# ulab-uiuc/UniRec

Hardware: AMD Instinct MI355X
Metric: user-sequences/sec joint fwd+bwd (Qwen3-0.6B+LoRA, hist=50) (higher is better)
Workload: dtype bf16; 1 GPU; C4 joint step: item Q-Former(L12,H1024,Q2,F14) on 64x50 items -> inject -> Qwen3-0.6B-shaped(28L)+LoRA r16 -> mean-pool -> InfoNCE pool 1000; fwd+bwd+allreduce+AdamW; per_gpu_batch=64, global_batch=64, seq_len=2048, hist=50, pool=1000, micro_batches=1, recompute_mlp=False, parallelism=dp1, random_init=True

## Files before the change

unirec_amd/csrc/gemm.hip:

```cpp
#include <cstdlib>
#include <type_traits>
#include "common.hip.h"
#include "unirec_hip.h"
#include "gemm_common.hip.h"

using urgemm::GemmP;
using urgemm::GemmPlan;
using urgemm::GemmGroups;
using urgemm::GemmGroupSlot;
using urgemm::UR_GEMM_MAX_GROUPS;
using urgemm::uniform_ptr;

namespace {

#ifndef UR_GEMM_STAMPS
#define UR_GEMM_STAMPS 0
#endif
#if UR_GEMM_STAMPS
__device__ long long g_gemm_stamps[8192 * 8];
#define UR_STAMP(k) do { if (threadIdx.x == 0 && blockIdx.x < 8192 && blockIdx.z == 0) g_gemm_stamps[blockIdx.x * 8 + (k)] = (long long)__builtin_readcyclecounter(); } while (0)
#else
#define UR_STAMP(k) do { } while (0)
#endif
constexpr int BK = 64;
// ... 218 lines not shown
    float4 a = w4[i];
    for (int z = 1; z < splits; ++z) {
      const float4 b = w4[i + (long)z * total4];
      a.x += b.x; a.y += b.y; a.z += b.z; a.w += b.w;
    }
    c4[i] = a;
  }
}

template <int BM, int BN, int NWM, int NWN>
int launch_grouped_cfg(const GemmP& p, const GemmGroups& gs, int nwg, int splits, hipStream_t st) {
  constexpr int SMEM = NSTAGE * (Tile<BN>::KS_BYTES + Tile<BM>::KS_BYTES);
  static std::atomic<uint64_t> attr_set{0};
  UR_ONCE_PER_DEVICE(attr_set) {
    hipError_t e = hipFuncSetAttribute(reinterpret_cast<const void*>(&gemm_grouped_kernel<false, false, true, BM, BN, NWM, NWN>),
                                       hipFuncAttributeMaxDynamicSharedMemorySize, SMEM);
    if (e != hipSuccess) UR_FAIL((int)e, "ur_gemm_grouped: hipFuncSetAttribute failed: %s", hipGetErrorString(e));
  }
  hipLaunchKernelGGL((gemm_grouped_kernel<false, false, true, BM, BN, NWM, NWN>), dim3(nwg, 1, splits), dim3(NWM * NWN * 64), SMEM, st, p, gs);
  UR_CHECK_LAUNCH("ur_gemm_grouped");
  return 0;
}

}

#if UR_GEMM_STAMPS
extern "C" int ur_lab_gemm_stamps(long long* host, int n) {
  return (int)hipMemcpyFromSymbol(host, HIP_SYMBOL(g_gemm_stamps), sizeof(long long) * n);
}
#endif

static void fill_params(const ur_gemm_args* a, GemmP& p) {
  p.R = (const bf16_t*)a->R; p.S = (const bf16_t*)a->S; p.ldr = a->ldr; p.lds = a->lds; p.K = a->K;
  p.R2 = (const bf16_t*)a->R2; p.S2 = (const bf16_t*)a->S2; p.ldr2 = a->ldr2; p.lds2 = a->lds2; p.K2 = a->K2;
  p.C = a->C; p.ldc = a->ldc; p.M = a->M; p.N = a->N; p.alpha = a->alpha;
  p.bias = a->bias; p.res = (const bf16_t*)a->residual; p.ldres = a->ldres;
  p.gelu_out = (bf16_t*)a->gelu_out; p.ldg = a->ldg; p.aux = (const bf16_t*)a->gelu_grad_aux; p.ldaux = a->ldaux;
  p.gm = 0; p.gn = 0;
  p.drop_bits = (const uint8_t*)a->drop_bits; p.drop_bits_ld = a->drop_bits_ld; p.drop_bits_stride = a->drop_bits_stride;
  p.drop_rank = a->drop_rank;
  p.drop_inv_keep = a->drop_bits ? 1.0f / (1.0f - a->drop_p) : 1.0f;
  p.sw_gu = (const bf16_t*)a->swiglu_gu; p.sw_ldgu = a->swiglu_ldgu; p.sw_dgu = (bf16_t*)a->swiglu_dgu; p.sw_lddgu = a->swiglu_lddgu;
  p.sw_I = a->swiglu_I; p.sw_mode = a->swiglu_gu ? 1 : 0;
  if (a->swiglu_gate) {
    p.sw_gu = (const bf16_t*)a->swiglu_gate; p.sw_ldgu = a->swiglu_ldgate; p.sw_dgu = (bf16_t*)a->swiglu_act; p.sw_lddgu = a->swiglu_ldact;
    p.sw_I = 0; p.sw_mode = 2;
  }
  p.qk_q = (bf16_t*)a->qkr_q; p.qk_ldq = a->qkr_ldq; p.qk_k = (bf16_t*)a->qkr_k; p.qk_ldk = a->qkr_ldk; p.qk_v = (bf16_t*)a->qkr_v; p.qk_ldv = a->qkr_ldv;
  p.qk_rstd = a->qkr_rstd; p.qk_qw = a->qkr_qw; p.qk_kw = a->qkr_kw; p.qk_cos = a->qkr_cos; p.qk_sin = a->qkr_sin;
  p.qk_S = a->qkr_S; p.qk_nq = a->qkr_nq_cols; p.qk_nk = a->qkr_nk_cols; p.qk_eps = a->qkr_eps;
  p.sp_act = (bf16_t*)a->swp_act; p.sp_ldact = a->swp_ldact; p.sp_I = a->swp_I;
  p.ksplit_len = 0; p.slab_stride = 0; p.gcw = 0; p.pad_ = 0;
}

static std::atomic<int> g_pers_mode{-1};
extern "C" int ur_gemm_persistent_mode(int mode) { return g_pers_mode.exchange(mode < 0 ? -1 : (mode > 2 ? 1 : mode)); }

static bool pers_takes(const GemmP& p, int splits, bool rk, bool sk, bool outf32) {
  constexpr int BM = 256, BN = 256;
  const int set = g_pers_mode.load(std::memory_order_relaxed);
  const int mode = set >= 0 ? set : 1;
  if (!mode || !rk || !sk || outf32 || splits > 1) return false;
  if ((p.M % BM) || (p.N % BN) || (p.K % BK) || p.K < 4 * BK) return false;
  constexpr int min_tiles = 128;
  if ((long)(p.M / BM) * (p.N / BN) < min_tiles) return false;
  if ((long)(p.M / BM) * (p.N / BN) >= (1L << 20) || p.N / BN >= (1 << 12) || p.M / BM >= (1 << 15)) return false;
  if (p.sw_mode == 2) return false;
  if (p.gelu_out || p.aux) {
    if ((p.gelu_out && p.aux) || p.res || p.K2 > 0 || p.sw_mode || p.qk_q || p.sp_act) return false;
    if (p.gelu_out && ((p.ldg & 7) || (reinterpret_cast<uintptr_t>(p.gelu_out) & 15))) return false;
    if (p.aux && ((p.ldaux & 7) || (reinterpret_cast<uintptr_t>(p.aux) & 15))) return false;
  }
  if (p.K2 > 0 && !p.drop_bits && p.K2 > BK) return false;
  if (p.drop_bits && p.K2 > 0) {
    if (p.drop_rank != 16 || (p.K2 & 15)) return false;
    constexpr int kmax = 8192;
    if (p.K > kmax) return false;
  }
  if (p.sw_mode == 1 && (p.bias || p.res)) return false;
  if ((p.ldc & 7) || (reinterpret_cast<uintptr_t>(p.C) & 15)) return false;
  if (p.res && ((p.ldres & 7) || (reinterpret_cast<uintptr_t>(p.res) & 15))) return false;
  if (p.sw_mode == 1 && ((p.sw_ldgu & 7) || (p.sw_lddgu & 7) || (p.sw_I & 7) || (reinterpret_cast<uintptr_t>(p.sw_gu) & 15) ||
                         (reinterpret_cast<uintptr_t>(p.sw_dgu) & 15))) return false;
  if (p.lds * 16 >= (1L << 31) || p.ldr * 16 >= (1L << 31) || p.ldc * 32 >= (1L << 31)) return false;
  auto wide = [](long ld) { return ld * 32 >= (1L << 31); };
  if ((p.res && wide(p.ldres)) || (p.sw_mode == 1 && (wide(p.sw_ldgu) || wide(p.sw_lddgu))) || (p.qk_q && (wide(p.qk_ldq) || wide(p.qk_ldk) || wide(p.qk_ldv))) ||
      (p.sp_act && wide(p.sp_ldact)) || (p.gelu_out && wide(p.ldg)) || (p.aux && wide(p.ldaux)) || (p.drop_bits && (wide(p.drop_bits_ld) || wide(p.lds2) || wide(p.ldr2))))
    return false;
  return true;
}

static GemmPlan gemm_select(const GemmP& p, int splits, bool rk, bool sk, bool outf32) {
  GemmPlan pl = {UR_GEMM_KERNEL_GENERIC, 128, 0, 0, 0, splits};
  if (pers_takes(p, splits, rk, sk, outf32)) {
    pl.kernel = UR_GEMM_KERNEL_PERSISTENT; pl.tile = 256;
    const int gm = p.M / 256, gn = p.N / 256;
    const int cw = (gn % 6) == 0 && gn >= 24 ? 6 : 4;
    if (gn >= 16 && (gm % 8) == 0 && gn > cw && (gn % cw) == 0) pl.gcw = cw;
    pl.mode = p.drop_bits != nullptr && p.K2 > 0 ? 2 : (p.K2 > 0 ? 1 : 0);
    pl.epi = p.sp_act ? 4 : (p.qk_q ? 3 : (p.sw_mode == 1 ? 1 : (p.gelu_out ? 6 : (p.aux ? 7 : (p.res ? 2 : (p.bias ? 5 : 0))))));
    return pl;
  }
  if (p.qk_q || p.sp_act) { pl.kernel = UR_GEMM_KERNEL_NONE; return pl; }
  if (rk && sk && !outf32) pl.epi = p.sw_mode;
  const long big_wgs = (long)ur_cdiv(p.M, 256) * ur_cdiv(p.N, 256) * splits;
  const long big_min = (!rk && !sk) ? 224 : 256;
  if (p.M >= 256 && p.N >= 256 && big_wgs >= big_min) pl.tile = 256;
  const int gm = ur_cdiv(p.M, pl.tile), gn = ur_cdiv(p.N, pl.tile);
  const int cw = gn >= 16 ? 4 : 0;
  if (cw > 0 && pl.tile == 256 && (gm % 8) == 0 && gn > cw && (gn % cw) == 0) pl.gcw = cw;
  return pl;
}

static GemmPlan gemm_select_grouped(const ur_gemm_args* a, int count) {
  const int splits = a->split_k > 1 ? a->split_k : 1;
  bool big = true;
  long t256 = 0;
  for (int i = 0; i < count; ++i) {
    big = big && a[i].M >= 256 && a[i].N >= 256;
    t256 += (long)ur_cdiv(a[i].M, 256) * ur_cdiv(a[i].N, 256);
  }
  big = big && t256 * splits >= 128;
  return GemmPlan{UR_GEMM_KERNEL_GROUPED, big ? 256 : 128, 0, 0, 0, splits};
}

static bool swiglu_paired_ok(const ur_gemm_args* a, const GemmPlan& pl) {
  if (a->swp_I <= 0 || a->N != 2 * a->swp_I || (a->swp_I % 128)) return false;
  if (a->bias || a->residual || a->gelu_out || a->gelu_grad_aux || a->drop_bits || a->swiglu_gu || a->swiglu_gate || a->qkr_q || a->alpha != 1.0f) return false;
  if ((a->swp_ldact & 7) || a->swp_ldact < a->swp_I || !UR_ALIGNED16(a->swp_act) || a->ldc < a->N) return false;
  return pl.kernel == UR_GEMM_KERNEL_PERSISTENT;
}

static bool qkrope_ok(const ur_gemm_args* a, const GemmPlan& pl) {
  if (!a->qkr_k || !a->qkr_v || !a->qkr_rstd || !a->qkr_qw || !a->qkr_kw || !a->qkr_cos || !a->qkr_sin) return false;
  if (a->bias || a->residual || a->gelu_out || a->gelu_grad_aux || a->drop_bits || a->swiglu_gu || a->swiglu_gate || a->alpha != 1.0f) return false;
  if (a->qkr_S < 256 || (a->qkr_S % 256) || (a->qkr_nq_cols % 256) || (a->qkr_nk_cols % 256) || a->qkr_nq_cols < 0 || a->qkr_nk_cols < 0 ||
      a->qkr_nq_cols + a->qkr_nk_cols > a->N || ((a->N - a->qkr_nq_cols - a->qkr_nk_cols) % 256)) return false;
  if ((a->qkr_ldq & 7) || (a->qkr_ldk & 7) || (a->qkr_ldv & 7) || !UR_ALIGNED16(a->qkr_q) || !UR_ALIGNED16(a->qkr_k) || !UR_ALIGNED16(a->qkr_v) ||
      !UR_ALIGNED16(a->qkr_qw) || !UR_ALIGNED16(a->qkr_kw) || !UR_ALIGNED16(a->qkr_cos) || !UR_ALIGNED16(a->qkr_sin)) return false;
  if (a->qkr_ldq < a->qkr_nq_cols || a->qkr_ldk < a->qkr_nk_cols || a->qkr_ldv < a->N - a->qkr_nq_cols - a->qkr_nk_cols) return false;
  return pl.kernel == UR_GEMM_KERNEL_PERSISTENT;
}

extern "C" int ur_qkrope_perm(int c) { return ((c >> 4) & 1) * 64 + ((c >> 5) & 3) * 16 + (c & 15); }

extern "C" int64_t ur_gemm_workspace_bytes(const ur_gemm_args* a) {
  if (!a || a->split_k <= 1) return 0;
  return (int64_t)a->split_k * a->M * a->ldc * (int64_t)sizeof(float);
}

static int gemm_check(const ur_gemm_args* a) {
  UR_REQUIRE(a != nullptr, "ur_gemm: null args");
  UR_REQUIRE(a->M >= 0 && a->N >= 0 && a->K >= 0 && a->K2 >= 0, "ur_gemm: negative dimension");
  if (a->M == 0 || a->N == 0) return 0;
  UR_REQUIRE(a->R && a->S && a->C, "ur_gemm: null operand");
  UR_REQUIRE((!a->r_kcontig && !a->s_kcontig) || ((a->K % 8) == 0 && (a->K2 % 8) == 0),
             "ur_gemm: K (%d) and K2 (%d) must be multiples of 8 for K-contiguous operands", a->K, a->K2);
  UR_REQUIRE((a->N % 4) == 0 && (a->ldc % 4) == 0, "ur_gemm: N (%d) and ldc (%ld) must be multiples of 4", a->N, (long)a->ldc);
  UR_REQUIRE((a->ldr % 8) == 0 && (a->lds % 8) == 0, "ur_gemm: ldr/lds must be multiples of 8 elements");
  UR_REQUIRE(a->r_kcontig || (a->M % 8) == 0, "ur_gemm: K-strided R needs M %% 8 == 0 (M=%d)", a->M);
  UR_REQUIRE(a->s_kcontig || (a->N % 8) == 0, "ur_gemm: K-strided S needs N %% 8 == 0 (N=%d)", a->N);
  UR_REQUIRE(UR_ALIGNED16(a->R) && UR_ALIGNED16(a->S) && UR_ALIGNED16(a->C), "ur_gemm: operands must be 16-byte aligned");
  UR_REQUIRE(a->ldr >= (a->r_kcontig ? a->K : a->M) && a->lds >= (a->s_kcontig ? a->K : a->N) && (a->ldc >= a->N || a->qkr_q),
             "ur_gemm: leading dimension smaller than row length");
  if (a->K2 > 0) {
    UR_REQUIRE(a->R2 && a->S2 && UR_ALIGNED16(a->R2) && UR_ALIGNED16(a->S2), "ur_gemm: bad second operand pair");
// ... 180 lines not shown
```

unirec_amd/csrc/gemm_pers.hip:

```cpp
#include <atomic>
#include <cstdlib>
#include <type_traits>
#include "gemm_common.hip.h"
#include "unirec_hip.h"

namespace {
using namespace urgemm;

#ifndef UR_PERS_STAMPS
#define UR_PERS_STAMPS 0
#endif
#if UR_PERS_STAMPS
__device__ long long g_pers_stamps[256 * 2 * 8];
#define UR_PSTAMP(k) do { if (tile_ord == UR_PERS_STAMPS && lane == 0 && (uwave & 3) == 0 && blockIdx.x < 256) g_pers_stamps[(blockIdx.x * 2 + (uwave >> 2)) * 8 + (k)] = (long long)__builtin_readcyclecounter(); } while (0)
#else
#define UR_PSTAMP(k) do { } while (0)
#endif
constexpr int BK = 64, BM = 256, BN = 256;
constexpr int S_BYTES = BN * 128, R_BYTES = BM * 128, STAGE = S_BYTES + R_BYTES;

template <int EPI, int MODE>
__global__ __launch_bounds__(512, 2) void gemm_pers_kernel(GemmP p, TileOrder ord, int ntiles) {
  constexpr bool DROP = MODE == 2, K2S = MODE == 1;
  constexpr bool REMAP = EPI != 3 && EPI != 4;
  extern __shared__ __attribute__((aligned(16))) char smem[];
  const int tid = threadIdx.x, lane = tid & 63;
  const int uwave = __builtin_amdgcn_readfirstlane(tid >> 6);
  const int wr = uwave >> 2, wc = uwave & 3;
  const int l15 = lane & 15, g4 = lane >> 4;
  const uint32_t lo0 = l15 * 128 + (((g4) ^ ((l15 >> 1) & 7)) << 4), lo1 = l15 * 128 + (((4 + g4) ^ ((l15 >> 1) & 7)) << 4);
  const int kch = (lane & 7) ^ (((lane >> 4) + 4 * (uwave & 1)) & 7);
  const uint32_t vo_s = (uint32_t)((lane >> 3) * p.lds * 2 + kch * 16), vo_r = (uint32_t)((lane >> 3) * p.ldr * 2 + kch * 16);
  const int nk1 = p.K / BK;
  const int nkt = nk1 + (K2S ? 1 : 0);
  const int gstride = gridDim.x;

  int vid = blockIdx.x, m0, n0;
  { int bm, bn; tile_coords(ord, vid, bm, bn); m0 = bm * BM; n0 = bn * BN; }
  int tiles_left = (ntiles - (int)blockIdx.x + gstride - 1) / gstride;
  auto s_base = [&](int n) { return reinterpret_cast<const char*>(p.S + (long)(n + (REMAP ? (uwave & 3) * 8 + (uwave >> 2) * 64 : uwave * 8)) * p.lds); };
  auto r_base = [&](int m) { return reinterpret_cast<const char*>(p.R + (long)(m + uwave * 8) * p.ldr); };
  const char* ubs = uniform_ptr(s_base(n0));
  const char* ubr = uniform_ptr(r_base(m0));
  const long sp_main = 64 * p.lds * 2, rp_main = 64 * p.ldr * 2;
  auto dma_half = [&](char* slot, auto is_s, int hf, auto zc) {
    constexpr bool IS_S = decltype(is_s)::value, Z = decltype(zc)::value;
#pragma unroll
    for (int d = 0; d < 2; ++d) {
      const int li = 2 * hf + d;
      char* dst = slot + (IS_S ? 0 : S_BYTES) + (li * 8 + uwave) * 1024;
      if constexpr (!Z) {
        const long s_off = REMAP ? (long)(d * 128 + hf * 32) * p.lds * 2 : li * sp_main;
        const char* src = (IS_S ? ubs + s_off : ubr + li * rp_main) + (IS_S ? vo_s : vo_r);
        __builtin_amdgcn_global_load_lds((gbl_void*)src, (lds_void*)dst, 16, 0, 0);
      } else {
        const long ld2 = IS_S ? p.lds2 : p.ldr2;
        const __amdgpu_buffer_rsrc_t rs = __builtin_amdgcn_make_buffer_rsrc(const_cast<char*>(IS_S ? ubs : ubr), 0, (int)(256 * ld2 * 2), 0x00020000);
        int zl = lane;
        asm volatile("" : "+v"(zl));
        const int zk = (zl & 7) ^ (((zl >> 4) + 4 * (uwave & 1)) & 7);
        const uint32_t vo = (zk * 8 < p.K2) ? (uint32_t)((zl >> 3) * ld2 * 2 + zk * 16) : 0x80000000u;
        __builtin_amdgcn_raw_ptr_buffer_load_lds(rs, (lds_void*)dst, 16, vo, (int)((IS_S && REMAP ? d * 128 + hf * 32 : li * 64) * ld2 * 2), 0, 0);
      }
    }
  };

  f32x4 acc[4][8];
  bf16x8 R0[4][2], R1[4][2], S0[2][2], S1[2][2];
  auto rdR = [&](bf16x8 (&F)[4][2], const char* slot, int rh) {
    const char* b = slot + S_BYTES + (rh * 128 + wr * 64) * 128;
#pragma unroll
    for (int jj = 0; jj < 4; ++jj) {
      F[jj][0] = *reinterpret_cast<const bf16x8*>(b + jj * 2048 + lo0);
      F[jj][1] = *reinterpret_cast<const bf16x8*>(b + jj * 2048 + lo1);
    }
  };
  auto rdS = [&](bf16x8 (&F)[2][2], const char* slot, int sh) {
    const char* b = slot + (sh * 128 + wc * 32) * 128;
#pragma unroll
    for (int ii = 0; ii < 2; ++ii) {
      F[ii][0] = *reinterpret_cast<const bf16x8*>(b + ii * 2048 + lo0);
      F[ii][1] = *reinterpret_cast<const bf16x8*>(b + ii * 2048 + lo1);
    }
  };
  auto quad = [&](const bf16x8 (&S)[2][2], const bf16x8 (&R)[4][2], auto shc, auto rhc, auto firstc) {
    constexpr int sh = decltype(shc)::value, rh = decltype(rhc)::value;
    constexpr bool FIRST = decltype(firstc)::value;
    __builtin_amdgcn_s_setprio(1);
#pragma unroll
    for (int h = 0; h < 2; ++h)
#pragma unroll
      for (int ii = 0; ii < 2; ++ii)
#pragma unroll
        for (int jj = 0; jj < 4; ++jj) {
          f32x4& a = acc[2 * sh + ii][4 * rh + jj];
          if (FIRST && h == 0) a = __builtin_amdgcn_mfma_f32_16x16x32_bf16(S[ii][h], R[jj][h], f32x4{0.f, 0.f, 0.f, 0.f}, 0, 0, 0);
          else a = __builtin_amdgcn_mfma_f32_16x16x32_bf16(S[ii][h], R[jj][h], a, 0, 0, 0);
        }
    __builtin_amdgcn_s_setprio(0);
  };
  auto mat_end = [&]() {
    __builtin_amdgcn_sched_barrier(0);
    __builtin_amdgcn_s_barrier();
    __builtin_amdgcn_sched_barrier(0);
  };
  const std::integral_constant<int, 0> c0;
  const std::integral_constant<int, 1> c1;
  auto ktile = [&](char* slot, const char* nslot, auto firstc, auto vmc, auto zc) {
    constexpr int VM = decltype(vmc)::value;
    auto seg_end = [&]() {
      __builtin_amdgcn_sched_barrier(0);
      asm volatile("s_waitcnt vmcnt(%0)" :: "n"(VM) : "memory");
      __builtin_amdgcn_s_waitcnt(0xc07f);
      __builtin_amdgcn_s_barrier();
      __builtin_amdgcn_sched_barrier(0);
    };
    rdS(S0, slot, 0);
    dma_half(slot, std::false_type{}, 0, zc);
    seg_end();
    quad(S0, R0, c0, c0, firstc);
    mat_end();
    rdS(S1, slot, 1);
    dma_half(slot, std::true_type{}, 0, zc);
    seg_end();
    quad(S1, R0, c1, c0, firstc);
    mat_end();
    rdR(R1, slot, 1);
    dma_half(slot, std::true_type{}, 1, zc);
    seg_end();
    quad(S1, R1, c1, c1, firstc);
    mat_end();
    rdR(R0, nslot, 0);
    dma_half(slot, std::false_type{}, 1, zc);
    seg_end();
    quad(S0, R1, c0, c1, firstc);
    mat_end();
  };

#pragma unroll 1
  for (int tt = 0; tt < 2; ++tt) {
    char* slot = smem + tt * STAGE;
    dma_half(slot, std::false_type{}, 0, std::false_type{}); __builtin_amdgcn_sched_barrier(0);
    dma_half(slot, std::true_type{}, 0, std::false_type{});  __builtin_amdgcn_sched_barrier(0);
    dma_half(slot, std::true_type{}, 1, std::false_type{});  __builtin_amdgcn_sched_barrier(0);
    dma_half(slot, std::false_type{}, 1, std::false_type{}); __builtin_amdgcn_sched_barrier(0);
    ubs = uniform_ptr(ubs + BK * 2); ubr = uniform_ptr(ubr + BK * 2);
  }
  asm volatile("s_waitcnt vmcnt(12)" ::: "memory");
  __builtin_amdgcn_s_barrier();
  __builtin_amdgcn_sched_barrier(0);
  rdR(R0, smem, 0);
  __builtin_amdgcn_s_waitcnt(0xc07f);
  __builtin_amdgcn_s_barrier();
  if (wr == 1) __builtin_amdgcn_s_barrier();
  __builtin_amdgcn_sched_barrier(0);

  int q = 0;
  bool first_tile = true;
#if UR_PERS_STAMPS
  int tile_ord = 0;
#endif
  const int sw = nkt - 2;
#pragma unroll 1
  for (;;) {
#if UR_PERS_STAMPS
    ++tile_ord;
#endif
    UR_PSTAMP(0);
    int nm0 = m0, nn0 = n0;
    if (tiles_left > 1) {
      vid += gstride;
      int bm, bn; tile_coords(ord, vid, bm, bn); nm0 = bm * BM; nn0 = bn * BN;
    }
    {
      char* slot = smem + (q & 1) * STAGE;
      const char* nslot = smem + ((q + 1) & 1) * STAGE;
      if (first_tile) ktile(slot, nslot, std::true_type{}, std::integral_constant<int, 12>{}, std::false_type{});
      else ktile(slot, nslot, std::true_type{}, std::integral_constant<int, 28>{}, std::false_type{});
      ++q;
      first_tile = false;
    }
    UR_PSTAMP(1);
    if constexpr (!K2S) {
#pragma unroll 1
      for (int kt = 1; kt < nkt; ++kt, ++q) {
        char* slot = smem + (q & 1) * STAGE;
        const char* nslot = smem + ((q + 1) & 1) * STAGE;
        if (kt == sw) { ubs = uniform_ptr(s_base(nn0)); ubr = uniform_ptr(r_base(nm0)); }
        else { ubs = uniform_ptr(ubs + BK * 2); ubr = uniform_ptr(ubr + BK * 2); }
        ktile(slot, nslot, std::false_type{}, std::integral_constant<int, 12>{}, std::false_type{});
#if UR_PERS_STAMPS
        if (kt <= 4) UR_PSTAMP(1 + kt);
#endif
      }
    } else {
#pragma unroll 1
      for (int kt = 1; kt < nk1 - 2; ++kt, ++q) {
        char* slot = smem + (q & 1) * STAGE;
        const char* nslot = smem + ((q + 1) & 1) * STAGE;
        ubs = uniform_ptr(ubs + BK * 2); ubr = uniform_ptr(ubr + BK * 2);
        ktile(slot, nslot, std::false_type{}, std::integral_constant<int, 12>{}, std::false_type{});
      }
      {
        char* slot = smem + (q & 1) * STAGE;
        const char* nslot = smem + ((q + 1) & 1) * STAGE;
        ubs = uniform_ptr(reinterpret_cast<const char*>(p.S2 + (long)(n0 + (REMAP ? (uwave & 3) * 8 + (uwave >> 2) * 64 : uwave * 8)) * p.lds2));
        ubr = uniform_ptr(reinterpret_cast<const char*>(p.R2 + (long)(m0 + uwave * 8) * p.ldr2));
        ktile(slot, nslot, std::false_type{}, std::integral_constant<int, 12>{}, std::true_type{});
        ++q;
      }
      ubs = uniform_ptr(s_base(nn0)); ubr = uniform_ptr(r_base(nm0));
#pragma unroll 1
      for (int kt = 0; kt < 2; ++kt, ++q) {
        char* slot = smem + (q & 1) * STAGE;
        const char* nslot = smem + ((q + 1) & 1) * STAGE;
        ktile(slot, nslot, std::false_type{}, std::integral_constant<int, 12>{}, std::false_type{});
        ubs = uniform_ptr(ubs + BK * 2); ubr = uniform_ptr(ubr + BK * 2);
      }
    }
    ubs = uniform_ptr(s_base(nn0) + 2 * BK * 2); ubr = uniform_ptr(r_base(nm0) + 2 * BK * 2);
    constexpr bool JOIN = DROP || EPI == 3;
    if (JOIN && wr == 0) __builtin_amdgcn_s_barrier();
    UR_PSTAMP(6);
    __builtin_amdgcn_sched_barrier(0);
    int elane = lane;
    asm volatile("" : "+v"(elane));
    const int el15 = elane & 15, eg4 = elane >> 4;
    if constexpr (DROP) {
      const int nad = p.K2 >> 4, kq = 4 * eg4;
      const uint32_t lo_s2 = (uint32_t)((el15 * p.lds2 + kq) * 2), lo_r2 = (uint32_t)((el15 * p.ldr2 + kq) * 2), lo_fl = (uint32_t)(el15 * p.drop_bits_ld);
      for (int a = 0; a < nad; ++a) {
        bf16x4 s2[4], r2[8];
        uint2 fl[8];
#pragma unroll
        for (int i = 0; i < 4; ++i) {
          const char* ub = uniform_ptr(reinterpret_cast<const char*>(p.S2 + (long)(n0 + (REMAP ? wc * 64 + (i >> 1) * 32 : (i >> 1) * 128 + wc * 32) + (i & 1) * 16) * p.lds2 + a * 16));
          s2[i] = ld_g<bf16x4>(ub + lo_s2);
        }
#pragma unroll
        for (int j = 0; j < 8; ++j) {
          const long mb = m0 + (j >> 2) * 128 + wr * 64 + (j & 3) * 16;
          const char* ub = uniform_ptr(reinterpret_cast<const char*>(p.R2 + mb * p.ldr2 + a * 16));
          r2[j] = ld_g<bf16x4>(ub + lo_r2);
          const char* fb = uniform_ptr(reinterpret_cast<const char*>(p.drop_bits + (long)a * p.drop_bits_stride + mb * p.drop_bits_ld + ((n0 + (REMAP ? wc * 64 : wc * 32)) >> 3)));
          fl[j] = make_uint2(ld_g<uint32_t>(fb + lo_fl), ld_g<uint32_t>(fb + lo_fl + (REMAP ? 4 : 16)));
        }
#pragma unroll
        for (int i = 0; i < 4; ++i)
#pragma unroll
          for (int j = 0; j < 8; ++j) {
            const f32x4 d = __builtin_amdgcn_mfma_f32_16x16x16bf16_1k(s2[i], r2[j], f32x4{0.f, 0.f, 0.f, 0.f}, 0, 0, 0);
            const uint32_t wsel = (i >= 2) ? fl[j].y : fl[j].x;
            const uint32_t f = (wsel >> (16 * (i & 1) + 8 * (eg4 >> 1) + 2 * (eg4 & 1))) & 0x33u;
            f32x4& c = acc[i][j];
            if (!(f & 0x01u)) c[0] += d[0] * p.drop_inv_keep;
            if (!(f & 0x10u)) c[1] += d[1] * p.drop_inv_keep;
            if (!(f & 0x02u)) c[2] += d[2] * p.drop_inv_keep;
            if (!(f & 0x20u)) c[3] += d[3] * p.drop_inv_keep;
          }
      }
    }
    if constexpr (EPI == 4) {
      const int cs = (eg4 & 1) * 16 + (eg4 >> 1) * 8;
      const int f0 = (n0 >> 1) + wc * 32 + cs;
      bf16_t* Cb = reinterpret_cast<bf16_t*>(p.C);
#pragma unroll
      for (int j = 0; j < 8; ++j) {
        const long m = m0 + (j >> 2) * 128 + wr * 64 + (j & 3) * 16 + el15;
        uint32_t gq[4], uq[4];
        {
          const f32x4 a = acc[0][j], b = acc[1][j];
          gq[0] = pack_bf2(a[0], a[1]); gq[1] = pack_bf2(a[2], a[3]); gq[2] = pack_bf2(b[0], b[1]); gq[3] = pack_bf2(b[2], b[3]);
          swap16(gq[0], gq[2]); swap16(gq[1], gq[3]);
        }
        {
          const f32x4 a = acc[2][j], b = acc[3][j];
          uq[0] = pack_bf2(a[0], a[1]); uq[1] = pack_bf2(a[2], a[3]); uq[2] = pack_bf2(b[0], b[1]); uq[3] = pack_bf2(b[2], b[3]);
          swap16(uq[0], uq[2]); swap16(uq[1], uq[3]);
        }
        uint32_t aq[4];
#pragma unroll
        for (int e = 0; e < 4; ++e) aq[e] = pack_bf2(silu_f(bf_lo(gq[e])) * bf_lo(uq[e]), silu_f(bf_hi(gq[e])) * bf_hi(uq[e]));
        const u32x4_t vg = {gq[0], gq[1], gq[2], gq[3]}, vu = {uq[0], uq[1], uq[2], uq[3]}, va = {aq[0], aq[1], aq[2], aq[3]};
        st_g<u32x4_t>(Cb + m * p.ldc + f0, vg);
        st_g<u32x4_t>(Cb + m * p.ldc + p.sp_I + f0, vu);
        st_g<u32x4_t>(p.sp_act + m * p.sp_ldact + f0, va);
      }
    } else
    if constexpr (EPI == 3) {
      const int qkc = p.qk_nq + p.qk_nk;
      if (n0 < qkc) {
        float* part = reinterpret_cast<float*>(smem + 2 * STAGE);
        const bool isq = n0 < p.qk_nq;
        const float* wgt = isq ? p.qk_qw : p.qk_kw;
        const int dq0 = wc * 16 + 4 * eg4;
        const int pos0 = m0 % p.qk_S;
        const int prow0 = pos0 + wr * 64 + el15;
        const float4 w0 = ld_g<float4>(wgt + dq0), w1 = ld_g<float4>(wgt + 64 + dq0);
        const float4 c_0 = ld_g<float4>(p.qk_cos + (long)prow0 * 64 + dq0), s_0 = ld_g<float4>(p.qk_sin + (long)prow0 * 64 + dq0);
        const float4 c16 = ld_g<float4>(p.qk_cos + 16 * 64 + dq0), s16 = ld_g<float4>(p.qk_sin + 16 * 64 + dq0);
        const float4 c80 = ld_g<float4>(p.qk_cos + 80 * 64 + dq0), s80 = ld_g<float4>(p.qk_sin + 80 * 64 + dq0);
#pragma unroll
        for (int sh = 0; sh < 2; ++sh)
#pragma unroll
          for (int j = 0; j < 8; ++j) {
            const f32x4 a = acc[2 * sh][j], b = acc[2 * sh + 1][j];
            float ss = a[0] * a[0] + a[1] * a[1] + a[2] * a[2] + a[3] * a[3] + b[0] * b[0] + b[1] * b[1] + b[2] * b[2] + b[3] * b[3];
            ss += __shfl_xor(ss, 16, 64);
            ss += __shfl_xor(ss, 32, 64);
            const int row = (j >> 2) * 128 + wr * 64 + (j & 3) * 16 + el15;
            if (eg4 == 0) part[(sh * 256 + row) * 4 + wc] = ss;
          }
        __syncthreads();
        bf16_t* outb = isq ? p.qk_q : p.qk_k;
        const long ldo = isq ? p.qk_ldq : p.qk_ldk;
        const int c0 = isq ? n0 : n0 - p.qk_nq;
        const int nheads = qkc >> 7, head0 = n0 >> 7;
        const int ocol = (eg4 & 1) * 64 + wc * 16 + (eg4 >> 1) * 8;
        float cv[4] = {c_0.x, c_0.y, c_0.z, c_0.w}, sv[4] = {s_0.x, s_0.y, s_0.z, s_0.w};
        const float wa[4] = {w0.x, w0.y, w0.z, w0.w}, wb[4] = {w1.x, w1.y, w1.z, w1.w};
        const float dc16[4] = {c16.x, c16.y, c16.z, c16.w}, ds16[4] = {s16.x, s16.y, s16.z, s16.w};
        const float dc80[4] = {c80.x, c80.y, c80.z, c80.w}, ds80[4] = {s80.x, s80.y, s80.z, s80.w};
#pragma unroll
        for (int j = 0; j < 8; ++j) {
          const int row = (j >> 2) * 128 + wr * 64 + (j & 3) * 16 + el15;
#pragma unroll
          for (int sh = 0; sh < 2; ++sh) {
            const float4 pr = *reinterpret_cast<const float4*>(part + (sh * 256 + row) * 4);
            const float rs = rsqrtf((pr.x + pr.y + pr.z + pr.w) * (1.0f / 128.0f) + p.qk_eps);
            const f32x4 a = acc[2 * sh][j], b = acc[2 * sh + 1][j];
            float o0[4], o1[4];
#pragma unroll
            for (int e = 0; e < 4; ++e) {
              const float xa = a[e] * rs * wa[e], xb = b[e] * rs * wb[e];
              o0[e] = xa * cv[e] - xb * sv[e];
              o1[e] = xb * cv[e] + xa * sv[e];
            }
            uint32_t a0 = pack_bf2(o0[0], o0[1]), a1 = pack_bf2(o0[2], o0[3]), b0 = pack_bf2(o1[0], o1[1]), b1 = pack_bf2(o1[2], o1[3]);
            swap16(a0, b0); swap16(a1, b1);
            const long m = m0 + row;
            const u32x4_t v = {a0, a1, b0, b1};
            st_g<u32x4_t>(outb + m * ldo + c0 + sh * 128 + ocol, v);
// ... 133 lines not shown
              for (int e = 0; e < 4; ++e) {
                g1[e] = pack_bf2(gelu_erf_f(bf_lo(z1[e])), gelu_erf_f(bf_hi(z1[e])));
                g2[e] = pack_bf2(gelu_erf_f(bf_lo(z2[e])), gelu_erf_f(bf_hi(z2[e])));
              }
              st_g<u32x4_t>(gb + log1, g1);
              st_g<u32x4_t>(gb + log2, g2);
            }
          }
        }
      } else {
        static_assert(EPI == 1, "the remaining epilogue is the SwiGLU backward");
        __builtin_amdgcn_sched_barrier(0);
        int em0 = __builtin_amdgcn_readfirstlane(m0), en0 = __builtin_amdgcn_readfirstlane(n0);
        asm volatile("" : "+s"(em0), "+s"(en0));
        uint4 gw[3][2], uw[3][2];
        uint32_t lg1, lg2, ld1, ld2;
        line_offs(p.sw_ldgu, lg1, lg2);
        line_offs(p.sw_lddgu, ld1, ld2);
        const long up_g = (long)p.sw_I * 2;
        auto load_block = [&](int j, uint4 (&g)[2], uint4 (&u)[2]) {
          const char* gb = uniform_ptr(reinterpret_cast<const char*>(p.sw_gu + (long)(em0 + (j >> 2) * 128 + wr * 64 + (j & 3) * 16) * p.sw_ldgu + en0 + wc * 64));
          g[0] = ld_g<uint4>(gb + lg1); g[1] = ld_g<uint4>(gb + lg2);
          u[0] = ld_g<uint4>(gb + up_g + lg1); u[1] = ld_g<uint4>(gb + up_g + lg2);
        };
        load_block(0, gw[0], uw[0]);
        load_block(1, gw[1], uw[1]);
#pragma unroll
        for (int j = 0; j < 8; ++j) {
          if (j + 2 < 8) load_block(j + 2, gw[(j + 2) % 3], uw[(j + 2) % 3]);
          char* db = uniform_wptr(reinterpret_cast<char*>(p.sw_dgu + (long)(em0 + (j >> 2) * 128 + wr * 64 + (j & 3) * 16) * p.sw_lddgu + en0 + wc * 64));
          float x[2][8];
#pragma unroll
          for (int sh = 0; sh < 2; ++sh) {
            f32x4 a = acc[2 * sh][j], b = acc[2 * sh + 1][j];
#pragma unroll
            for (int e = 0; e < 4; ++e) { float xx = a[e], yy = b[e]; swap16f(xx, yy); a[e] = xx; b[e] = yy; }
#pragma unroll
            for (int e = 0; e < 4; ++e) { x[sh][e] = a[e] * alpha; x[sh][4 + e] = b[e] * alpha; }
          }
#pragma unroll
          for (int pos = 0; pos < 2; ++pos) {
            float v[8];
#pragma unroll
            for (int e = 0; e < 8; ++e)
              v[e] = pos ? __int_as_float(__builtin_amdgcn_update_dpp(__float_as_int(x[0][e]), __float_as_int(x[1][e]), 0x128, 0xf, 0x3, false))
                         : __int_as_float(__builtin_amdgcn_update_dpp(__float_as_int(x[0][e]), __float_as_int(x[1][e]), 0x128, 0xf, 0xc, false));
            const uint4 gq4 = gw[j % 3][pos], uq4 = uw[j % 3][pos];
            const uint32_t gq[4] = {gq4.x, gq4.y, gq4.z, gq4.w}, uq[4] = {uq4.x, uq4.y, uq4.z, uq4.w};
            uint32_t og[4], ou[4];
#pragma unroll
            for (int e = 0; e < 4; ++e) {
              float dgv[2], duv[2];
#pragma unroll
              for (int hh = 0; hh < 2; ++hh) {
                const float gg = hh ? bf_hi(gq[e]) : bf_lo(gq[e]), uu = hh ? bf_hi(uq[e]) : bf_lo(uq[e]);
                const float d = v[2 * e + hh];
                const float sg = sigmoid_f(gg);
                duv[hh] = d * (gg * sg);
                dgv[hh] = d * uu * (sg * (1.0f + gg * (1.0f - sg)));
              }
              og[e] = pack_bf2(dgv[0], dgv[1]); ou[e] = pack_bf2(duv[0], duv[1]);
            }
            const u32x4_t vg = {og[0], og[1], og[2], og[3]}, vu = {ou[0], ou[1], ou[2], ou[3]};
            st_g<u32x4_t>(db + (pos ? ld2 : ld1), vg);
            st_g<u32x4_t>(db + up_g + (pos ? ld2 : ld1), vu);
          }
        }
      }
    }
    __builtin_amdgcn_sched_barrier(0);
    UR_PSTAMP(7);
    if (JOIN && wr == 1 && tiles_left > 1) __builtin_amdgcn_s_barrier();
    tiles_left -= 1;
    if (tiles_left == 0) break;
    m0 = nm0; n0 = nn0;
  }
  if (!(DROP || EPI == 3) && wr == 0) __builtin_amdgcn_s_barrier();
  asm volatile("s_waitcnt vmcnt(0)" ::: "memory");
}

template <int EPI, int MODE>
int launch_pers(const GemmP& p, hipStream_t st) {
  static std::atomic<uint64_t> attr_set{0};
  constexpr int SMEM = 2 * STAGE + (EPI == 3 ? 2 * 256 * 4 * (int)sizeof(float) : 0);
  UR_ONCE_PER_DEVICE(attr_set) {
    hipError_t e = hipFuncSetAttribute(reinterpret_cast<const void*>(&gemm_pers_kernel<EPI, MODE>), hipFuncAttributeMaxDynamicSharedMemorySize, SMEM);
    if (e != hipSuccess) UR_FAIL((int)e, "ur_gemm(persistent): hipFuncSetAttribute failed: %s", hipGetErrorString(e));
  }
  int ncu = ur_device_cu_count();
  ncu -= ncu % 8;
  if (ncu <= 0) ncu = 8;
  const int ntiles = p.gm * p.gn;
  const int grid = ntiles < ncu ? ntiles : ncu;
  auto magic = [](int d) { return (uint32_t)(((1ull << 32) + (unsigned)d - 1) / (unsigned)d); };
  TileOrder o;
  o.nwg = ntiles; o.gn = p.gn; o.gcw = p.gcw;
  o.rows_x = (ntiles >> 3) / p.gn; o.per = o.rows_x * (p.gcw > 0 ? p.gcw : 1);
  o.m_gn = magic(p.gn); o.m_per = magic(o.per > 0 ? o.per : 1); o.m_gcw = magic(p.gcw > 0 ? p.gcw : 1);
  hipLaunchKernelGGL((gemm_pers_kernel<EPI, MODE>), dim3(grid), dim3(512), SMEM, st, p, o, ntiles);
  UR_CHECK_LAUNCH("ur_gemm(persistent)");
  return 0;
}

}

namespace urgemm {

int gemm_pers_launch(GemmP p, const GemmPlan& pl, hipStream_t st) {
  p.gm = p.M / BM; p.gn = p.N / BN; p.gcw = pl.gcw;
#define UR_PERS_CASE(E, MD) if (pl.epi == E && pl.mode == MD) return launch_pers<E, MD>(p, st)
  UR_PERS_CASE(0, 0); UR_PERS_CASE(0, 1); UR_PERS_CASE(0, 2);
  UR_PERS_CASE(1, 0); UR_PERS_CASE(1, 1); UR_PERS_CASE(1, 2);
  UR_PERS_CASE(2, 0); UR_PERS_CASE(2, 1); UR_PERS_CASE(2, 2);
  UR_PERS_CASE(3, 0); UR_PERS_CASE(3, 1);
  UR_PERS_CASE(4, 0); UR_PERS_CASE(4, 1);
  UR_PERS_CASE(5, 0); UR_PERS_CASE(5, 1); UR_PERS_CASE(5, 2);
  UR_PERS_CASE(6, 0); UR_PERS_CASE(7, 0);
#undef UR_PERS_CASE
  UR_FAIL(-1, "ur_gemm(persistent): no kernel for epilogue %d, mode %d", pl.epi, pl.mode);
}

}

#if UR_PERS_STAMPS
extern "C" int ur_lab_pers_stamps(long long* host, int n) {
  return (int)hipMemcpyFromSymbol(host, HIP_SYMBOL(g_pers_stamps), sizeof(long long) * n);
}
#endif
```

Before: 156.3 user-sequences/sec.

## Stage LoRA-dropout low-rank operands through LDS and prefetch them during the main K loop

In the persistent GEMM's dropout low-rank mode, the R2, S2 and dropout-flag loads that used to go straight from global memory into registers in the epilogue now land in an extra LDS zone. The first adapter slice is fetched during the last K tiles of the main loop, and later slices are double-buffered while the previous slice's MFMAs run. The goal is to hide the global latency of the rank-16 correction behind the main GEMM. In exchange it uses 32 KiB more LDS, adds barriers and hand-tuned vmcnt waits, and adds alignment checks that can send some shapes back to the generic kernel.

```diff
diff --git a/unirec_amd/csrc/gemm.hip b/unirec_amd/csrc/gemm.hip
--- a/unirec_amd/csrc/gemm.hip
+++ b/unirec_amd/csrc/gemm.hip
@@ -324,6 +324,8 @@
   if (p.res && ((p.ldres & 7) || (reinterpret_cast<uintptr_t>(p.res) & 15))) return false;
   if (p.sw_mode == 1 && ((p.sw_ldgu & 7) || (p.sw_lddgu & 7) || (p.sw_I & 7) || (reinterpret_cast<uintptr_t>(p.sw_gu) & 15) ||
                          (reinterpret_cast<uintptr_t>(p.sw_dgu) & 15))) return false;
+  if (p.drop_bits && p.K2 > 0 && ((p.ldr2 & 7) || (p.lds2 & 7) || (reinterpret_cast<uintptr_t>(p.R2) & 15) || (reinterpret_cast<uintptr_t>(p.S2) & 15) ||
+                                  (p.drop_bits_stride & 15))) return false;
   if (p.lds * 16 >= (1L << 31) || p.ldr * 16 >= (1L << 31) || p.ldc * 32 >= (1L << 31)) return false;
   auto wide = [](long ld) { return ld * 32 >= (1L << 31); };
   if ((p.res && wide(p.ldres)) || (p.sw_mode == 1 && (wide(p.sw_ldgu) || wide(p.sw_lddgu))) || (p.qk_q && (wide(p.qk_ldq) || wide(p.qk_ldk) || wide(p.qk_ldv))) ||
diff --git a/unirec_amd/csrc/gemm_pers.hip b/unirec_amd/csrc/gemm_pers.hip
--- a/unirec_amd/csrc/gemm_pers.hip
+++ b/unirec_amd/csrc/gemm_pers.hip
@@ -18,6 +18,7 @@
 #endif
 constexpr int BK = 64, BM = 256, BN = 256;
 constexpr int S_BYTES = BN * 128, R_BYTES = BM * 128, STAGE = S_BYTES + R_BYTES;
+constexpr int ZONE = 4 * 8192, Z_S2 = 0, Z_R2X = 8192, Z_FLX = 16384, Z_R2Y = 24576, Z_FLY = 0;
 
 template <int EPI, int MODE>
 __global__ __launch_bounds__(512, 2) void gemm_pers_kernel(GemmP p, TileOrder ord, int ntiles) {
@@ -51,7 +52,9 @@
       char* dst = slot + (IS_S ? 0 : S_BYTES) + (li * 8 + uwave) * 1024;
       if constexpr (!Z) {
         const long s_off = REMAP ? (long)(d * 128 + hf * 32) * p.lds * 2 : li * sp_main;
-        const char* src = (IS_S ? ubs + s_off : ubr + li * rp_main) + (IS_S ? vo_s : vo_r);
+        uint32_t vo = IS_S ? vo_s : vo_r;
+        if constexpr (DROP) asm volatile("" : "+v"(vo));
+        const char* src = (IS_S ? ubs + s_off : ubr + li * rp_main) + vo;
         __builtin_amdgcn_global_load_lds((gbl_void*)src, (lds_void*)dst, 16, 0, 0);
       } else {
         const long ld2 = IS_S ? p.lds2 : p.ldr2;
@@ -106,36 +109,38 @@
   };
   const std::integral_constant<int, 0> c0;
   const std::integral_constant<int, 1> c1;
-  auto ktile = [&](char* slot, const char* nslot, auto firstc, auto vmc, auto zc) {
-    constexpr int VM = decltype(vmc)::value;
-    auto seg_end = [&]() {
+  auto ktile_x = [&](char* slot, const char* nslot, auto firstc, auto vmc, auto vmc2, auto zc, auto&& extra) {
+    auto seg_end = [&](auto vm) {
+      constexpr int VM = decltype(vm)::value;
       __builtin_amdgcn_sched_barrier(0);
       asm volatile("s_waitcnt vmcnt(%0)" :: "n"(VM) : "memory");
       __builtin_amdgcn_s_waitcnt(0xc07f);
       __builtin_amdgcn_s_barrier();
       __builtin_amdgcn_sched_barrier(0);
     };
+    extra();
     rdS(S0, slot, 0);
     dma_half(slot, std::false_type{}, 0, zc);
-    seg_end();
+    seg_end(vmc);
     quad(S0, R0, c0, c0, firstc);
     mat_end();
     rdS(S1, slot, 1);
     dma_half(slot, std::true_type{}, 0, zc);
-    seg_end();
+    seg_end(vmc);
     quad(S1, R0, c1, c0, firstc);
     mat_end();
     rdR(R1, slot, 1);
     dma_half(slot, std::true_type{}, 1, zc);
-    seg_end();
+    seg_end(vmc2);
     quad(S1, R1, c1, c1, firstc);
     mat_end();
     rdR(R0, nslot, 0);
     dma_half(slot, std::false_type{}, 1, zc);
-    seg_end();
+    seg_end(vmc2);
     quad(S0, R1, c0, c1, firstc);
     mat_end();
   };
+  auto ktile = [&](char* slot, const char* nslot, auto firstc, auto vmc, auto zc) { ktile_x(slot, nslot, firstc, vmc, vmc, zc, [] {}); };
 
 #pragma unroll 1
   for (int tt = 0; tt < 2; ++tt) {
@@ -181,7 +186,42 @@
       first_tile = false;
     }
     UR_PSTAMP(1);
-    if constexpr (!K2S) {
+    if constexpr (DROP) {
+#pragma unroll 1
+      for (int kt = 1; kt < nkt - 2; ++kt, ++q) {
+        char* slot = smem + (q & 1) * STAGE;
+        const char* nslot = smem + ((q + 1) & 1) * STAGE;
+        ubs = uniform_ptr(ubs + BK * 2); ubr = uniform_ptr(ubr + BK * 2);
+        ktile(slot, nslot, std::false_type{}, std::integral_constant<int, 12>{}, std::false_type{});
+      }
+      auto stage0 = [&]() {
+        int zl = lane;
+        asm volatile("" : "+v"(zl));
+        const int zr = zl >> 1, zh = (zl & 1) * 16;
+        char* z = smem + 2 * STAGE + uwave * 1024;
+        const char* us = uniform_ptr(reinterpret_cast<const char*>(p.S2 + (long)(n0 + uwave * 32) * p.lds2));
+        const char* ur = uniform_ptr(reinterpret_cast<const char*>(p.R2 + (long)(m0 + uwave * 32) * p.ldr2));
+        const char* uf = uniform_ptr(reinterpret_cast<const char*>(p.drop_bits + (long)(m0 + uwave * 32) * p.drop_bits_ld + (n0 >> 3)));
+        __builtin_amdgcn_global_load_lds((gbl_void*)(us + (uint32_t)(zr * (int)(p.lds2 * 2) + zh)), (lds_void*)(z + Z_S2), 16, 0, 0);
+        __builtin_amdgcn_global_load_lds((gbl_void*)(ur + (uint32_t)(zr * (int)(p.ldr2 * 2) + zh)), (lds_void*)(z + Z_R2X), 16, 0, 0);
+        __builtin_amdgcn_global_load_lds((gbl_void*)(uf + (uint32_t)(zr * (int)p.drop_bits_ld + zh)), (lds_void*)(z + Z_FLX), 16, 0, 0);
+        __builtin_amdgcn_sched_barrier(0);
+      };
+      {
+        char* slot = smem + (q & 1) * STAGE;
+        const char* nslot = smem + ((q + 1) & 1) * STAGE;
+        ubs = uniform_ptr(s_base(nn0)); ubr = uniform_ptr(r_base(nm0));
+        ktile_x(slot, nslot, std::false_type{}, std::integral_constant<int, 15>{}, std::integral_constant<int, 15>{}, std::false_type{}, stage0);
+        ++q;
+      }
+      {
+        char* slot = smem + (q & 1) * STAGE;
+        const char* nslot = smem + ((q + 1) & 1) * STAGE;
+        ubs = uniform_ptr(ubs + BK * 2); ubr = uniform_ptr(ubr + BK * 2);
+        ktile_x(slot, nslot, std::false_type{}, std::integral_constant<int, 15>{}, std::integral_constant<int, 12>{}, std::false_type{}, [] {});
+        ++q;
+      }
+    } else if constexpr (!K2S) {
 #pragma unroll 1
       for (int kt = 1; kt < nkt; ++kt, ++q) {
         char* slot = smem + (q & 1) * STAGE;
@@ -220,44 +260,77 @@
     }
     ubs = uniform_ptr(s_base(nn0) + 2 * BK * 2); ubr = uniform_ptr(r_base(nm0) + 2 * BK * 2);
     constexpr bool JOIN = DROP || EPI == 3;
+    if constexpr (DROP) asm volatile("s_waitcnt vmcnt(14)" ::: "memory");
     if (JOIN && wr == 0) __builtin_amdgcn_s_barrier();
+    if constexpr (DROP) __builtin_amdgcn_s_barrier();
     UR_PSTAMP(6);
     __builtin_amdgcn_sched_barrier(0);
     int elane = lane;
     asm volatile("" : "+v"(elane));
     const int el15 = elane & 15, eg4 = elane >> 4;
     if constexpr (DROP) {
+      static_assert(REMAP, "the flag words of a wave's two 32-column groups are one 8-byte read");
       const int nad = p.K2 >> 4, kq = 4 * eg4;
-      const uint32_t lo_s2 = (uint32_t)((el15 * p.lds2 + kq) * 2), lo_r2 = (uint32_t)((el15 * p.ldr2 + kq) * 2), lo_fl = (uint32_t)(el15 * p.drop_bits_ld);
+      const uint32_t zb = lds_off(smem + 2 * STAGE);
+      const uint32_t za_s2 = zb + Z_S2 + (uint32_t)((wc * 64 + el15) * 32 + kq * 2);
+      const uint32_t za_r2 = zb + (uint32_t)((wr * 64 + el15) * 32 + kq * 2), za_fl = zb + (uint32_t)((wr * 64 + el15) * 32 + wc * 8);
+      bf16x4 s2[4];
+      asm volatile("ds_read_b64 %0, %4\n\tds_read_b64 %1, %4 offset:512\n\tds_read_b64 %2, %4 offset:1024\n\tds_read_b64 %3, %4 offset:1536\n\t"
+                   "s_waitcnt lgkmcnt(0)"
+                   : "=&v"(s2[0]), "=&v"(s2[1]), "=&v"(s2[2]), "=&v"(s2[3]) : "v"(za_s2) : "memory");
+      auto load_s2 = [&](bf16x4 (&dst)[4], int ad) {
+        const uint32_t lo_s2 = (uint32_t)((el15 * p.lds2 + kq) * 2);
+#pragma unroll
+        for (int i = 0; i < 4; ++i) {
+          const char* ub = uniform_ptr(reinterpret_cast<const char*>(p.S2 + (long)(n0 + wc * 64 + (i >> 1) * 32 + (i & 1) * 16) * p.lds2 + ad * 16));
+          dst[i] = ld_g<bf16x4>(ub + lo_s2);
+        }
+      };
       for (int a = 0; a < nad; ++a) {
-        bf16x4 s2[4], r2[8];
-        uint2 fl[8];
-#pragma unroll
-        for (int i = 0; i < 4; ++i) {
-          const char* ub = uniform_ptr(reinterpret_cast<const char*>(p.S2 + (long)(n0 + (REMAP ? wc * 64 + (i >> 1) * 32 : (i >> 1) * 128 + wc * 32) + (i & 1) * 16) * p.lds2 + a * 16));
-          s2[i] = ld_g<bf16x4>(ub + lo_s2);
-        }
-#pragma unroll
-        for (int j = 0; j < 8; ++j) {
-          const long mb = m0 + (j >> 2) * 128 + wr * 64 + (j & 3) * 16;
-          const char* ub = uniform_ptr(reinterpret_cast<const char*>(p.R2 + mb * p.ldr2 + a * 16));
-          r2[j] = ld_g<bf16x4>(ub + lo_r2);
-          const char* fb = uniform_ptr(reinterpret_cast<const char*>(p.drop_bits + (long)a * p.drop_bits_stride + mb * p.drop_bits_ld + ((n0 + (REMAP ? wc * 64 : wc * 32)) >> 3)));
-          fl[j] = make_uint2(ld_g<uint32_t>(fb + lo_fl), ld_g<uint32_t>(fb + lo_fl + (REMAP ? 4 : 16)));
-        }
-#pragma unroll
-        for (int i = 0; i < 4; ++i)
-#pragma unroll
-          for (int j = 0; j < 8; ++j) {
-            const f32x4 d = __builtin_amdgcn_mfma_f32_16x16x16bf16_1k(s2[i], r2[j], f32x4{0.f, 0.f, 0.f, 0.f}, 0, 0, 0);
-            const uint32_t wsel = (i >= 2) ? fl[j].y : fl[j].x;
-            const uint32_t f = (wsel >> (16 * (i & 1) + 8 * (eg4 >> 1) + 2 * (eg4 & 1))) & 0x33u;
-            f32x4& c = acc[i][j];
-            if (!(f & 0x01u)) c[0] += d[0] * p.drop_inv_keep;
-            if (!(f & 0x10u)) c[1] += d[1] * p.drop_inv_keep;
-            if (!(f & 0x02u)) c[2] += d[2] * p.drop_inv_keep;
-            if (!(f & 0x20u)) c[3] += d[3] * p.drop_inv_keep;
-          }
+        const bool more = a + 1 < nad;
+        if (more) {
+          if (a == 0) __builtin_amdgcn_s_barrier();
+          const int zr = elane >> 1, zh = (elane & 1) * 16;
+          char* z = smem + 2 * STAGE + uwave * 1024;
+          const char* ur = uniform_ptr(reinterpret_cast<const char*>(p.R2 + (long)(m0 + uwave * 32) * p.ldr2 + (a + 1) * 16));
+          const char* uf = uniform_ptr(reinterpret_cast<const char*>(p.drop_bits + (long)(a + 1) * p.drop_bits_stride + (long)(m0 + uwave * 32) * p.drop_bits_ld + (n0 >> 3)));
+          __builtin_amdgcn_global_load_lds((gbl_void*)(ur + (uint32_t)(zr * (int)(p.ldr2 * 2) + zh)), (lds_void*)(z + ((a & 1) ? Z_R2X : Z_R2Y)), 16, 0, 0);
+          __builtin_amdgcn_global_load_lds((gbl_void*)(uf + (uint32_t)(zr * (int)p.drop_bits_ld + zh)), (lds_void*)(z + ((a & 1) ? Z_FLX : Z_FLY)), 16, 0, 0);
+          __builtin_amdgcn_sched_barrier(0);
+        }
+        const uint32_t ar = za_r2 + ((a & 1) ? Z_R2Y : Z_R2X), af = za_fl + ((a & 1) ? Z_FLY : Z_FLX);
+#pragma unroll
+        for (int jp = 0; jp < 4; ++jp) {
+          bf16x4 r2[2];
+          u32x2_t fl[2];
+          const uint32_t jo = (uint32_t)((jp >> 1) * 4096 + (jp & 1) * 1024);
+          asm volatile("ds_read_b64 %0, %4\n\tds_read_b64 %1, %4 offset:512\n\tds_read_b64 %2, %5\n\tds_read_b64 %3, %5 offset:512\n\t"
+                       "s_waitcnt lgkmcnt(0)"
+                       : "=&v"(r2[0]), "=&v"(r2[1]), "=&v"(fl[0]), "=&v"(fl[1]) : "v"(ar + jo), "v"(af + jo) : "memory");
+#pragma unroll
+          for (int jj = 0; jj < 2; ++jj)
+#pragma unroll
+            for (int i = 0; i < 4; ++i) {
+              const int j = 2 * jp + jj;
+              const f32x4 d = __builtin_amdgcn_mfma_f32_16x16x16bf16_1k(s2[i], r2[jj], f32x4{0.f, 0.f, 0.f, 0.f}, 0, 0, 0);
+              const uint32_t wsel = (i >= 2) ? fl[jj].y : fl[jj].x;
+              const uint32_t f = (wsel >> (16 * (i & 1) + 8 * (eg4 >> 1) + 2 * (eg4 & 1))) & 0x33u;
+              f32x4& c = acc[i][j];
+              if (!(f & 0x01u)) c[0] += d[0] * p.drop_inv_keep;
+              if (!(f & 0x10u)) c[1] += d[1] * p.drop_inv_keep;
+              if (!(f & 0x02u)) c[2] += d[2] * p.drop_inv_keep;
+              if (!(f & 0x20u)) c[3] += d[3] * p.drop_inv_keep;
+              asm volatile("" : "+v"(c));
+            }
+        }
+        if (more) {
+          load_s2(s2, a + 1);
+          __builtin_amdgcn_sched_barrier(0);
+          asm volatile("s_waitcnt vmcnt(0)" ::: "memory");
+          __builtin_amdgcn_s_barrier();
+          asm volatile("" : "+v"(s2[0]), "+v"(s2[1]), "+v"(s2[2]), "+v"(s2[3]));
+          __builtin_amdgcn_sched_barrier(0);
+        }
       }
     }
     if constexpr (EPI == 4) {
@@ -557,7 +630,9 @@
 template <int EPI, int MODE>
 int launch_pers(const GemmP& p, hipStream_t st) {
   static std::atomic<uint64_t> attr_set{0};
-  constexpr int SMEM = 2 * STAGE + (EPI == 3 ? 2 * 256 * 4 * (int)sizeof(float) : 0);
+  static_assert(!(EPI == 3 && MODE == 2), "the row sums of EPI 3 and the landing zone of MODE 2 share the LDS behind the ring");
+  constexpr int SMEM = 2 * STAGE + (EPI == 3 ? 2 * 256 * 4 * (int)sizeof(float) : 0) + (MODE == 2 ? ZONE : 0);
+  static_assert(SMEM <= 160 * 1024, "a CU has 160 KiB of LDS");
   UR_ONCE_PER_DEVICE(attr_set) {
     hipError_t e = hipFuncSetAttribute(reinterpret_cast<const void*>(&gemm_pers_kernel<EPI, MODE>), hipFuncAttributeMaxDynamicSharedMemorySize, SMEM);
     if (e != hipSuccess) UR_FAIL((int)e, "ur_gemm(persistent): hipFuncSetAttribute failed: %s", hipGetErrorString(e));
```

Result: no change. 157.8 user-sequences/sec, median of 6 (+1.0%).
